# kfjahnke/envutil

Measured on AMD Instinct MI355X. Metric: Mpix/s reprojected (16K lat/lon->cubemap, b-spline-3), higher is better.
Workload: dtype f32

## Files before the change

envutil_amd/csrc/eu_render4.hip:

```cpp
#include <cstdio>
#include <cstring>
#include <vector>
#include <algorithm>
#include "eu_packed_dev.h"
#include "eu_launch.h"

#define EU4_TW 16
#define EU4_TH 8
#define EU4_WAVES 4
#ifndef EU4_WAVES0
#define EU4_WAVES0 1
#define EU4_TEXELS 384
#define EU4_OCC0 4
#endif
#define EU4_SHARDS 1024
#define EU4_WL_SHARD(s) (16 * (s))
#define EU4_WL_DONE1 (16 * EU4_SHARDS)
#define EU4_WL_DYN(x) (16 * (EU4_SHARDS + 1 + (x)))
#define EU4_WL_ENTRIES (16 * (EU4_SHARDS + 16))
#define EU4_UNIT_ROWS 4
#define EU4_COL_FLOATS 8
#define EU4_MAX_PLANS 16

__device__ __forceinline__ void eu4_box_reduce(int &mn0, int &mn1, int &mx0, int &mx1)
// ... 27 lines not shown
  unsigned keep;
  asm volatile("s_mov_b32 %0, m0\n\t"
               "s_mov_b32 m0, %1\n\t"
               "s_nop 0\n\t"
               "global_load_lds_dwordx4 %2, %3\n\t"
               "s_mov_b32 m0, %0"
               : "=&s"(keep) : "s"(dst), "v"(voff), "s"(sb) : "memory");
}

struct eu4_plan {
  const float *atab_g;
  const int *tileplan;
  const float *coltab;
  int tiles16;
  const int *l2_rows;
  int l2_off[9];
  int l2_half;
  unsigned long long l2_magic;
  const int *l1_ent;
  int l1_off[9];
  int l1_ecols;
  unsigned long long l1_magic;
  const int *xtab;
#ifdef EU5_STAMPS
  unsigned long long *stamps;
#endif
};

#ifdef EU5_STAMPS
#define EU5_STAMP(k) do { asm volatile("" ::: "memory"); st_[k] = __builtin_amdgcn_s_memtime(); asm volatile("" ::: "memory"); } while (0)
#define EU5_STAMP32(k) do { asm volatile("" ::: "memory"); st_[k] = (unsigned)__builtin_amdgcn_s_memtime(); asm volatile("" ::: "memory"); } while (0)
#else
#define EU5_STAMP(k) do { } while (0)
#define EU5_STAMP32(k) do { } while (0)
#endif

template <int NCH, int DEG, int PRJ>
__device__ __forceinline__ void eu4_tile(const eu_render_params &p, const eu4_plan &w, const float *atab,
                                         float *wtile, int tile_y, int x0, int lane)
{
  constexpr int TEX = 4;
  constexpr int order = DEG + 1;
  const eu_src_dev &s = p.src;
  const int lx = lane & 7, ly = lane >> 3;
  const int y = p.row_begin + tile_y * EU4_TH + ly;
  const bool yin = y < p.row_end;
// ... 252 lines not shown
  const int sh = gid & (EU4_SHARDS - 1);
  const int nwork = __builtin_amdgcn_readfirstlane(
    __hip_atomic_load(p.wl + EU4_WL_SHARD(sh), __ATOMIC_RELAXED, __HIP_MEMORY_SCOPE_AGENT));
  __syncthreads();
#pragma unroll 1
  for (int k = gid / EU4_SHARDS; k < nwork; k += (int)(gridDim.x * EU4_WAVES / EU4_SHARDS)) {
    const int id = __builtin_amdgcn_readfirstlane(p.wl[EU4_WL_ENTRIES + (size_t)k * EU4_SHARDS + sh]);
    const int tile_y = id / w.tiles16;
    const int x0 = (id - tile_y * w.tiles16) * EU4_TW;
    eu4_direct_tile<NCH, DEG, PRJ>(p, atab, tile_y, x0, lane);
  }
  __shared__ int last;
  __syncthreads();
  if (threadIdx.x == 0) last = atomicAdd(p.wl + EU4_WL_DONE1, 1) == (int)gridDim.x - 1;
  __syncthreads();
  if (last) {
    for (int i = threadIdx.x; i <= EU4_SHARDS + 8; i += 256)
      __hip_atomic_store(p.wl + 16 * i, 0, __ATOMIC_RELAXED, __HIP_MEMORY_SCOPE_AGENT);
  }
}

static long long eu4_followers_plan = 0, eu4_followers_last = 0;
extern "C" unsigned long long eu_hip_share_follower_tiles(void) { return (unsigned long long)eu4_followers_last; }

#ifndef EU4_DIRECT_WGS
#define EU4_DIRECT_WGS 2048
#endif

template <int NCH, int DEG, int PRJ>
static int launch4_ndp(const eu_render_params &p, const eu4_plan &w, hipStream_t st)
{
  if constexpr (PRJ == EU_SPHERICAL) {
    static const int cus = [] {
      int dev = 0, n = 0;
      if (hipGetDevice(&dev) != hipSuccess) return 0;
      if (hipDeviceGetAttribute(&n, hipDeviceAttributeMultiprocessorCount, dev) != hipSuccess) return 0;
      return n;
    }();
    const bool fast = eu_staged_fast_profile(p);
    int per_cu = 0;
    if (fast) {
      static const int occ = [] { int n = 0; return hipOccupancyMaxActiveBlocksPerMultiprocessor(&n, eu_render5_kernel<NCH, DEG, PRJ, true>, 64 * EU5_WAVES, 0) == hipSuccess ? n : 0; }();
      per_cu = occ;
    } else {
      static const int occ = [] { int n = 0; return hipOccupancyMaxActiveBlocksPerMultiprocessor(&n, eu_render5_kernel<NCH, DEG, PRJ, false>, 64 * EU5_WAVES, 0) == hipSuccess ? n : 0; }();
      per_cu = occ;
    }
    const int wgs = (cus / 8) * 8 * per_cu;
    if (wgs <= 0) return -1;
    if (fast) eu4_followers_last = eu4_followers_plan;
    if (fast) hipLaunchKernelGGL((eu_render5_kernel<NCH, DEG, PRJ, true>), dim3((unsigned)wgs), dim3(64 * EU5_WAVES), 0, st, p, w);
    else hipLaunchKernelGGL((eu_render5_kernel<NCH, DEG, PRJ, false>), dim3((unsigned)wgs), dim3(64 * EU5_WAVES), 0, st, p, w);
  } else {
    const int units = (p.tiles_y + EU4_UNIT_ROWS - 1) / EU4_UNIT_ROWS;
    dim3 grid((unsigned)(8 * ((w.tiles16 + EU4_WAVES0 - 1) / EU4_WAVES0)), (unsigned)EU4_UNIT_ROWS, (unsigned)((units + 7) / 8));
    hipLaunchKernelGGL((eu_render4s_kernel<NCH, DEG, PRJ>), grid, dim3(64 * EU4_WAVES0), 0, st, p, w);
  }
  if (hipGetLastError() != hipSuccess) return -1;
  hipLaunchKernelGGL((eu_render4d_kernel<NCH, DEG, PRJ>), dim3(EU4_DIRECT_WGS), dim3(256), 0, st, p, w);
  if (hipGetLastError() != hipSuccess) {
    (void)hipMemsetAsync(p.wl, 0, EU4_WL_ENTRIES * sizeof(int), st);
    return -1;
  }
  return 0;
}

template <int NCH, int DEG>
static int launch4_nd(const eu_render_params &p, const eu4_plan &w, hipStream_t st)
{
  switch (p.src.prj) {
    case EU_SPHERICAL: return launch4_ndp<NCH, DEG, EU_SPHERICAL>(p, w, st);
    case EU_CUBEMAP: return launch4_ndp<NCH, DEG, EU_CUBEMAP>(p, w, st);
    case EU_BIATAN6: return launch4_ndp<NCH, DEG, EU_BIATAN6>(p, w, st);
  }
// ... 1 lines not shown
}

template <int NCH>
static int launch4_n(const eu_render_params &p, const eu4_plan &w, hipStream_t st)
{
  switch (p.src.degree) {
    case 1: return launch4_nd<NCH, 1>(p, w, st);
    case 2: return launch4_nd<NCH, 2>(p, w, st);
    case 3: return launch4_nd<NCH, 3>(p, w, st);
  }
  return -2;
}

extern "C" size_t eu_render4_worklist_ints(size_t ntiles)
{
  return EU4_WL_ENTRIES + ((ntiles + EU4_SHARDS - 1) / EU4_SHARDS) * EU4_SHARDS;
}
extern "C" size_t eu_render4_worklist_header_ints(void) { return EU4_WL_ENTRIES; }

static_assert(EU_STAGED_TILE_ROWS == EU4_TH && EU_STAGED_MAX_TILES_Y == 65535 * 8 * EU4_UNIT_ROWS, "eu_select.h: eu_staged_covers");
namespace {
struct plan_cache {
  std::vector<unsigned char> key;
  eu_dev_buf<int> tileplan, l2_rows, l1_ent, xtab;
  eu_dev_buf<float> coltab;
  float *atab = nullptr;
  int planned_rows = 0;
  int l2_off[9] = {};
  int l1_off[9] = {};
  int l1_ecols = 1;
  long long follower_tiles = 0;
  hipStream_t last_stream = nullptr;
} g4s[EU_MAX_SLOTS];
#define g4 (g4s[eu_current_slot()])

bool ensure_atab()
{
  if (g4.atab) return true;
  std::vector<float> tab(768, 0.0f);
  for (int i = 0; i < EU_ATAN_TAB_ENTRIES; i++) eu_atan_tab_entry(i, tab.data() + 8 * i);
  if (hipMalloc((void **)&g4.atab, tab.size() * sizeof(float)) != hipSuccess) return false;
  return hipMemcpy(g4.atab, tab.data(), tab.size() * sizeof(float), hipMemcpyHostToDevice) == hipSuccess;
}

template <int DEG>
void launch_colplan(const eu_render_params &p, float *ct, const float *k, hipStream_t st)
{
  hipLaunchKernelGGL((eu_colplan_kernel<DEG>), dim3((unsigned)((p.width + 511) / 512)), dim3(256), 0, st, p, ct,
                     k[0], k[1], k[2], k[3]);
}

std::vector<unsigned char> eu4_plan_key(const eu_render_params &p, unsigned long long plan_gen, int share_mode)
{
  std::vector<unsigned char> key(sizeof(unsigned long long) + sizeof(eu_src_dev) + 9 * sizeof(int));
  unsigned char *q = key.data();
  memcpy(q, &plan_gen, sizeof plan_gen); q += sizeof plan_gen;
  eu_src_dev sd = p.src; sd.base = nullptr;
  memcpy(q, &sd, sizeof sd); q += sizeof sd;
  const int v[9] = { p.width, p.row_begin, p.row_end, p.band_shift, p.band_count, p.band_index, p.form, p.norm_mode, share_mode };
  memcpy(q, v, sizeof v);
  return key;
}

bool upload(eu_dev_buf<int> &buf, const std::vector<int> &v, size_t spare)
{
  if (buf.reserve(v.size() + spare) != hipSuccess) return false;
  return v.empty() || hipMemcpy(buf.p, v.data(), v.size() * sizeof(int), hipMemcpyHostToDevice) == hipSuccess;
}

int eu4_build_plans(const eu_render_params &p, int tiles16, const eu_switches &sw, const float *h_row,
                    size_t h_row_floats, hipStream_t st)
{
  std::vector<int> tp((size_t)p.tiles_y, -1);
  std::vector<float> plans;
  const bool can = p.form == EU_FORM_BA && p.norm_mode == EU_NORM_NONE && h_row;
  if (can && sw.colplan) {
    for (int ty = 0; ty < p.tiles_y; ty++) {
      float k[4] = { 0, 0, 0, 0 };
      bool same = true;
      for (int ly = 0; ly < EU4_TH && same; ly++) {
        const int y = std::min(p.row_begin + ty * EU4_TH + ly, p.row_end - 1);
        const size_t fr = (size_t)eu_frame_row(y, p.band_shift, p.band_count, p.band_index) * EU_ROW_FLOATS;
        if (fr + 6 > h_row_floats) { same = false; break; }
        const float c[4] = { h_row[fr + 0], h_row[fr + 2], h_row[fr + 3], h_row[fr + 5] };
        if (ly == 0) memcpy(k, c, sizeof k);
        else same = memcmp(k, c, sizeof k) == 0;
      }
      if (!same) continue;
      int id = -1;
      for (size_t j = 0; j < plans.size() / 4 && id < 0; j++)
// ... 2 lines not shown
        id = (int)(plans.size() / 4);
        plans.insert(plans.end(), k, k + 4);
      }
      tp[(size_t)ty] = id;
    }
  }
  const int nplans = (int)(plans.size() / 4);
  if (g4.tileplan.reserve(tp.size()) != hipSuccess) return -1;
  if (g4.coltab.reserve(std::max<size_t>(1, nplans) * (size_t)p.width * EU4_COL_FLOATS) != hipSuccess) return -1;
  if (hipStreamSynchronize(st) != hipSuccess) return -1;
  if (g4.last_stream && g4.last_stream != st && hipStreamSynchronize(g4.last_stream) != hipSuccess) return -1;
  if (hipMemcpy(g4.tileplan.p, tp.data(), tp.size() * sizeof(int), hipMemcpyHostToDevice) != hipSuccess) return -1;
  g4.planned_rows = 0;
  for (int v : tp) g4.planned_rows += v >= 0;
  auto paired = [&](int m) { return 2 * m + 1 < p.tiles_y && tp[(size_t)2 * m] >= 0 && tp[(size_t)2 * m] == tp[(size_t)2 * m + 1]; };
  {
    std::vector<int> rows[8], all;
    for (int r = 0; r < p.tiles_y; r++)
      if (!paired(r >> 1)) rows[(r / EU5_UNIT_ROWS) & 7].push_back(r);
    for (int x = 0; x < 8; x++) { g4.l2_off[x] = (int)all.size(); all.insert(all.end(), rows[x].begin(), rows[x].end()); }
    g4.l2_off[8] = (int)all.size();
    if (!upload(g4.l2_rows, all, 1)) return -1;
  }
  for (int j = 0; j < nplans; j++) {
    float *ct = g4.coltab.p + j * (size_t)p.width * EU4_COL_FLOATS;
    switch (p.src.degree) {
      case 1: launch_colplan<1>(p, ct, &plans[4 * j], st); break;
      case 2: launch_colplan<2>(p, ct, &plans[4 * j], st); break;
      default: launch_colplan<3>(p, ct, &plans[4 * j], st); break;
    }
    if (hipGetLastError() != hipSuccess) return -1;
  }
  std::vector<float> h_ct((size_t)nplans * p.width * EU4_COL_FLOATS);
  if (nplans) {
    if (hipStreamSynchronize(st) != hipSuccess) return -1;
    if (hipMemcpy(h_ct.data(), g4.coltab.p, h_ct.size() * sizeof(float), hipMemcpyDeviceToHost) != hipSuccess) return -1;
  }
  std::vector<int> cm, cp;
  for (int m = 0; 2 * m + 1 < p.tiles_y; m++)
    if (paired(m)) { cm.push_back(m); cp.push_back(tp[(size_t)2 * m]); }
  eu_share_input in;
  in.width = p.width; in.tiles16 = tiles16; in.row_begin = p.row_begin; in.row_end = p.row_end;
  in.band_mode = p.band_count > 1;
  in.ncand = (int)cm.size(); in.cand_m = cm.data(); in.cand_plan = cp.data();
  in.h_row = h_row; in.h_row_floats = h_row_floats; in.row_floats = EU_ROW_FLOATS;
  in.coltab = nplans ? h_ct.data() : nullptr; in.col_floats = EU4_COL_FLOATS; in.nplans = nplans;
// ... 2 lines not shown
  eu_share_build(in, gr);
  if (!upload(g4.l1_ent, gr.entries, 2)) return -1;
  if (g4.xtab.reserve(gr.xtab.size()) != hipSuccess) return -1;
  if (hipMemcpy(g4.xtab.p, gr.xtab.data(), gr.xtab.size() * sizeof(int), hipMemcpyHostToDevice) != hipSuccess) return -1;
  for (int x = 0; x < 9; x++) g4.l1_off[x] = gr.off[x];
  g4.l1_ecols = gr.ecols;
  g4.follower_tiles = gr.follower_tiles;
  return 0;
}

void eu4_fill_plan(eu4_plan &w)
{
  w.tileplan = g4.tileplan.p;
  w.coltab = g4.coltab.p;
  w.l2_rows = g4.l2_rows.p;
  for (int x = 0; x < 9; x++) w.l2_off[x] = g4.l2_off[x];
  w.l2_half = (w.tiles16 + 1) / 2;
  w.l2_magic = (1ull << 40) / (unsigned long long)w.l2_half + 1;
  w.l1_ent = g4.l1_ent.p;
  for (int x = 0; x < 9; x++) w.l1_off[x] = g4.l1_off[x];
  w.l1_ecols = g4.l1_ecols;
  w.l1_magic = (1ull << 40) / (unsigned long long)w.l1_ecols + 1;
  w.xtab = g4.xtab.p;
}

int launch4(const eu_render_params &p, const eu4_plan &w, hipStream_t st)
{
  switch (p.nch) {
    case 3: return launch4_n<3>(p, w, st);
    case 4: return launch4_n<4>(p, w, st);
  }
  return -2;
}

#ifdef EU5_STAMPS
int launch4_stamped(const eu_render_params &p, eu4_plan &w, hipStream_t st)
{
  static unsigned long long *d_st = nullptr; static size_t st_cap = 0; static int dumps = 0;
  const size_t ntile_st = (size_t)w.tiles16 * p.tiles_y * 8;
  const size_t nst = ntile_st + 8192 * 4;
  if (st_cap < nst) { if (d_st) (void)hipFree(d_st); if (hipMalloc((void **)&d_st, nst * 8) != hipSuccess) return -1; st_cap = nst; }
  (void)hipMemsetAsync(d_st, 0, nst * 8, st);
  w.stamps = d_st;
  const int rc_ = launch4(p, w, st);
  if (rc_ == 0 && dumps < 2 && nst >= 8 * 4096) {
    dumps++;
// ... 16 lines not shown
        const unsigned long long *q = &h[ntile_st + k * 4];
        if (!q[3]) continue;
        const double d = (double)(q[2] - q[0]);
        mn = std::min(mn, d); mx = std::max(mx, d); sum += d; l1 += (double)(q[1] - q[0]); nw++;
        first = std::min(first, (double)q[0]); last = std::max(last, (double)q[2]);
      }
      if (nw) fprintf(stderr, "eu5 waves: %zu, cycles per wave min %.0f avg %.0f max %.0f, first loop avg %.0f, first start .. last end %.0f\n",
                      nw, mn, sum / nw, mx, l1 / nw, last - first);
    }
    for (int c = 0; c < 32; c++) if (cnt[c])
      fprintf(stderr, "eu5 stamps: hoist %d npass %2d tiles %8zu | coords %7.0f box %6.0f dma-issue+weights %6.0f dma-wait %6.0f taps(all passes) %6.0f store %5.0f | tile %7.0f (100 MHz ticks? s_memtime)\n",
              c >> 4, (c & 15) - 1, cnt[c], acc[c][0] / cnt[c], acc[c][1] / cnt[c], acc[c][2] / cnt[c], acc[c][3] / cnt[c], acc[c][4] / cnt[c], acc[c][5] / cnt[c], acc[c][6] / cnt[c]);
  }
  return rc_;
}
#endif
}

extern "C" int eu_launch_render4(const eu_render_params *pp, const eu_switches *sw, const float *h_row, size_t h_row_floats,
                                 unsigned long long plan_gen, void *stream, int *launches)
{
  eu_render_params p = *pp;
  eu4_followers_last = 0;
  *launches = 2;
  if (!eu_staged_covers(p) || !p.wl) return -2;
  p.tiles_y = (p.row_end - p.row_begin + EU4_TH - 1) / EU4_TH;
  eu4_plan w;
  w.tiles16 = (p.width + EU4_TW - 1) / EU4_TW;
  if (w.tiles16 <= 0 || p.tiles_y <= 0) return 0;
  hipStream_t st = (hipStream_t)stream;
  if (!ensure_atab()) return -1;
  w.atab_g = g4.atab;
  if (p.src.prj == EU_SPHERICAL) {
    std::vector<unsigned char> key = eu4_plan_key(p, plan_gen, sw->share);
    if (key != g4.key) {
      if (eu4_build_plans(p, w.tiles16, *sw, h_row, h_row_floats, st)) return -1;
      g4.key.swap(key);
    }
    if (sw->r4 != 1 && !eu_staged_worth(p.src.degree, g4.planned_rows, p.tiles_y)) { *launches = 0; return 0; }
  }
  eu4_fill_plan(w);
  eu4_followers_plan = g4.follower_tiles;
  g4.last_stream = st;
#ifdef EU5_STAMPS
  return launch4_stamped(p, w, st);
#else
  return launch4(p, w, st);
#endif
}
```

envutil_amd/csrc/eu_render5.h:

```cpp
#define EU5_WAVES 4
#ifndef EU5_TEXELS
#define EU5_TEXELS 576
#endif
#ifndef EU5_OCC
#define EU5_OCC 4
#endif
#ifndef EU5_UNIT_ROWS
#define EU5_UNIT_ROWS 4
#endif

__device__ __forceinline__ int eu4_shard_of(int id)
{
  return (int)(((unsigned)id * 0x9E3779B1u) >> 22) & (EU4_SHARDS - 1);
}

typedef const __attribute__((address_space(3))) eu4_f4 *eu5_l4ptr;

template <int NCH, int DEG>
__device__ __forceinline__ void eu5_taps(eu_lptr lt, int a, int b, int pitch, const eu_f2 *wx, const eu_f2 *wy,
                                         eu_f2 tx, eu_f2 ty, eu_f2 &rga, eu_f2 &bxa, eu_f2 &rgb, eu_f2 &bxb)
{
  constexpr int order = DEG + 1;
  if constexpr (DEG == 1) {
    const eu_f2 wl0 = 1.0f - tx, wr0 = tx, wl1 = 1.0f - ty, wr1 = ty;
// ... 106 lines not shown
  return cc + lower;
}

__device__ __forceinline__ int eu5_out_of_range3(float a, float b, float c)
{
  const float hi = __builtin_fmaxf(__builtin_fmaxf(__builtin_fabsf(a), __builtin_fabsf(b)), __builtin_fabsf(c));
  const float lo = __builtin_fminf(__builtin_fminf(__builtin_fabsf(a), __builtin_fabsf(b)), __builtin_fabsf(c));
  return (hi <= 0x1p40f && lo >= 0x1p-40f) ? 0 : -1;
}

struct eu5_tab8 { eu_f2 c0; float A0, A1, A2, B0, B1, B2; };

template <bool FAST>
__device__ __forceinline__ void eu5_load8(const eu_render_params &p, int tile_y, int x0, int lane, eu5_tab8 &T)
{
  const int pr = lane & 3, rw = (lane >> 2) & 7, hf = lane >> 5;
  const int y = p.row_begin + tile_y * EU4_TH + rw;
  const int yc = y < p.row_end ? y : p.row_end - 1;
  const float *rt = p.row + (long long)(FAST ? yc : eu_frame_row(yc, p.band_shift, p.band_count, p.band_index)) * EU_ROW_FLOATS;
  const int xa = x0 + 8 * hf + 2 * pr, xb = xa + 1;
  const int xac = xa < p.width ? xa : p.width - 1, xbc = xb < p.width ? xb : p.width - 1;
  T.A0 = rt[0]; T.A1 = rt[1]; T.A2 = rt[2]; T.B0 = rt[3]; T.B1 = rt[4]; T.B2 = rt[5];
  T.c0 = (eu_f2){ p.col[xac], p.col[xbc] };
}

template <int NCH, int DEG, int PRJ, bool HOIST, bool FAST, bool PRE = false>
__device__ __forceinline__ void eu5_tile(const eu_render_params &p, const eu4_plan &w, const float *atab,
                                         float *wtile, const float *ct, int tile_y, int x0, int lane,
                                         const eu5_tab8 *T = nullptr, bool have_n = false, int ty_n = 0, int x0_n = 0,
                                         eu5_tab8 *Tn = nullptr)
{
  static_assert(!PRE || (!HOIST && FAST), "the prefetching form exists for plain FAST tiles");
  constexpr int TEX = 4;
  constexpr int order = DEG + 1;
  const eu_src_dev &s = p.src;
#ifdef EU5_STAMPS
  unsigned long long st_[8] = { 0, 0, 0, 0, 0, 0, 0, 0 };
#endif
  EU5_STAMP(0);
  const int pr = lane & 3, rw = (lane >> 2) & 7, hf = lane >> 5;
  const int y = p.row_begin + tile_y * EU4_TH + rw;
  const bool yin = y < p.row_end;
  const int yc = yin ? y : p.row_end - 1;
  const float *rt = p.row + (long long)(FAST ? yc : eu_frame_row(yc, p.band_shift, p.band_count, p.band_index)) * EU_ROW_FLOATS;
  const int xa = x0 + 8 * hf + 2 * pr, xb = xa + 1;
  const bool va = yin && xa < p.width, vb = yin && xb < p.width;
// ... 262 lines not shown
__device__ __forceinline__ void eu5_stage(const eu_src_dev &s, const eu5_box &bx, unsigned lds_tile, int lane)
{
  constexpr int order = DEG + 1;
  const int ibw = bx.mxx - bx.mnx + order, ibh = bx.mxy - bx.mny + order;
  const unsigned tv = eu5_divtab.v[ibw];
  const int k = (int)(tv >> 24);
  const unsigned r = ((unsigned)lane * (tv & 0x1ffffu)) >> 16, c = (unsigned)lane - r * (unsigned)ibw;
  const int bx0 = bx.mnx - DEG / 2, by0 = bx.mny - DEG / 2;
  const unsigned pitchb = (unsigned)(s.es1 * 4);
  const unsigned voff = r * pitchb + c * (NCH * 4u);
  const char *const sb0 = (const char *)(s.base + ((long long)by0 * s.es1 + (long long)bx0 * NCH));
  const unsigned long long step = (unsigned long long)k * pitchb;
  const unsigned dstep = (unsigned)(k * ibw) * 16u;
  if ((int)r < k) {
    const char *sb = sb0;
    unsigned dst = lds_tile;
#pragma unroll 1
    for (int left = ibh; left >= k; left -= k) { eu4_dma_row(dst, voff, sb); sb += step; dst += dstep; }
  }
  if ((int)r < ibh % k) {
    const int full = ibh / k;
    eu4_dma_row(lds_tile + (unsigned)full * dstep, voff, sb0 + (unsigned long long)full * step);
  }
}

struct eu5_tab16 {
  eu4_f4 a0, a1, b0, b1;
  eu_f2 c0;
  float A1A, B1A, A1B, B1B;
};

__device__ __forceinline__ void eu5_load16(const eu_render_params &p, const float *ct, int tile_y, int x0, int lane, eu5_tab16 &T)
{
  const int pr = lane & 3, rw = (lane >> 2) & 7, hf = lane >> 5;
  const int yA = p.row_begin + tile_y * EU4_TH + rw, yB = yA + EU4_TH;
  const int ycA = yA < p.row_end ? yA : p.row_end - 1, ycB = yB < p.row_end ? yB : p.row_end - 1;
  const float *rtA = p.row + (long long)ycA * EU_ROW_FLOATS, *rtB = p.row + (long long)ycB * EU_ROW_FLOATS;
  const int xa = x0 + 8 * hf + 2 * pr, xb = xa + 1;
  const int xac = xa < p.width ? xa : p.width - 1, xbc = xb < p.width ? xb : p.width - 1;
  const eu4_f4 *ea = (const eu4_f4 *)(ct + (size_t)xac * EU4_COL_FLOATS);
  const eu4_f4 *eb = (const eu4_f4 *)(ct + (size_t)xbc * EU4_COL_FLOATS);
  T.a0 = ea[0]; T.a1 = ea[1]; T.b0 = eb[0]; T.b1 = eb[1];
  T.A1A = rtA[1]; T.B1A = rtA[4]; T.A1B = rtB[1]; T.B1B = rtB[4];
  T.c0 = (eu_f2){ p.col[xac], p.col[xbc] };
}

// ... 199 lines not shown
    rx += dx; ry += dy; ul += du;
    if (rx >= tiles16) { rx -= tiles16; ry++; }
    if (ry >= UNIT) { ry -= UNIT; ul++; }
  }
  __device__ __forceinline__ bool done() const { return ul * 8 + xcd >= units; }
  __device__ __forceinline__ int row() const { return (ul * 8 + xcd) * UNIT + ry; }
  __device__ __forceinline__ int col() const
  {
    const unsigned h = ((unsigned)row() * 0x9E3779B1u) >> 16;
    int c = rx + (int)((h * (unsigned)tiles16) >> 16);
    if (c >= tiles16) c -= tiles16;
    return c;
  }
};

__device__ __forceinline__ int eu5_pair_plan(const int *tileplan, int tiles_y, int m)
{
  if (2 * m + 1 >= tiles_y) return -1;
  const eu5_cint tp = (eu5_cint)tileplan;
  const int a = tp[2 * m], b = tp[2 * m + 1];
  return a == b ? a : -1;
}

template <int NCH, int DEG, int PRJ, bool FAST>
__global__ __launch_bounds__(64 * EU5_WAVES, EU5_OCC) void eu_render5_kernel(const eu_render_params p, const eu4_plan w)
{
  __shared__ __attribute__((aligned(16))) float tile_all[EU5_WAVES * EU5_TEXELS * 4];
  __shared__ __attribute__((aligned(16))) float atab[768];
  const int lane0 = threadIdx.x & 63;
  const int wave = __builtin_amdgcn_readfirstlane(threadIdx.x >> 6);
  float *const tile = tile_all + wave * (EU5_TEXELS * 4);
  if (PRJ != EU_CUBEMAP && wave == 0) {
#pragma unroll
    for (int i = 0; i < 3; i++)
      __builtin_amdgcn_global_load_lds((eu4_gbl_void)(w.atab_g + i * 256 + lane0 * 4),
                                       (eu4_lds_void)(atab + i * 256), 16, 0, 0);
    asm volatile("s_waitcnt vmcnt(0)" ::: "memory");
  }
  __syncthreads();
#ifdef EU5_STAMPS
  const unsigned long long ws0 = __builtin_amdgcn_s_memtime();
  unsigned long long ws1 = ws0;
#endif
  const int xcd = (int)(blockIdx.x & 7);
  const int K = (int)(gridDim.x >> 3) * EU5_WAVES;
  const int t0 = (int)(blockIdx.x >> 3) * EU5_WAVES + wave;
  constexpr bool PAIRS = FAST && PRJ == EU_SPHERICAL;
// ... 21 lines not shown
#pragma unroll 1
    while (have_a) {
      const bool have_n = seek(e_n, n_n, m_n, plan_n, col_n);
      eu5_group16<NCH, DEG>(p, w, atab, tile, T, e_a, n_a, m_a, plan_a, col_a, lane0, have_n, m_n, have_n ? plan_n : 0, col_n);
      e_a = e_n; n_a = n_n; m_a = m_n; plan_a = plan_n; col_a = col_n; have_a = have_n;
    }
  }
#ifdef EU5_STAMPS
  ws1 = __builtin_amdgcn_s_memtime();
#endif
  eu5_iter<EU5_UNIT_ROWS> it;
  it.xcd = xcd; it.tiles16 = w.tiles16;
  it.units = (p.tiles_y + EU5_UNIT_ROWS - 1) / EU5_UNIT_ROWS;
  it.start(t0, K);
  if constexpr (PAIRS) {
    int *const queue = p.wl + EU4_WL_DYN(xcd);
    const int nbatch = (w.l2_off[xcd + 1] - w.l2_off[xcd]) * w.l2_half;
    const eu5_cint rows2 = (eu5_cint)w.l2_rows + w.l2_off[xcd];
    auto take = [&]() -> int {
      int v = 0;
      if (lane0 == 0) v = atomicAdd(queue, 1);
      return v;
    };
    auto decode = [&](int j, int &ty, int &tcol) -> bool {
      if (j >= nbatch) return false;
      const int r = (int)(((unsigned long long)(unsigned)j * w.l2_magic) >> 40);
      ty = rows2[r]; tcol = 2 * (j - r * w.l2_half);
      return true;
    };
    int ty_a = 0, col_a = 0, ty_n = 0, col_n = 0;
    bool have = decode(__builtin_amdgcn_readfirstlane(take()), ty_a, col_a);
    eu5_tab8 Ta, Tb;
    if (have) eu5_load8<FAST>(p, ty_a, col_a * EU4_TW, lane0, Ta);
#pragma unroll 1
    while (have) {
      const int jn_lane = take();
      const bool second = col_a + 1 < w.tiles16;
      {
        int lane = lane0;
        asm volatile("" : "+v"(lane));
        eu5_tile<NCH, DEG, PRJ, false, FAST, true>(p, w, atab, tile, nullptr, ty_a, col_a * EU4_TW, lane, &Ta, second, ty_a,
                                                   (col_a + 1) * EU4_TW, &Tb);
      }
      const bool have_n = decode(__builtin_amdgcn_readfirstlane(jn_lane), ty_n, col_n);
      if (second) {
        int lane = lane0;
        asm volatile("" : "+v"(lane));
        eu5_tile<NCH, DEG, PRJ, false, FAST, true>(p, w, atab, tile, nullptr, ty_a, (col_a + 1) * EU4_TW, lane, &Tb, have_n, ty_n,
                                                   col_n * EU4_TW, &Ta);
      } else if (have_n) eu5_load8<FAST>(p, ty_n, col_n * EU4_TW, lane0, Ta);
      ty_a = ty_n; col_a = col_n; have = have_n;
    }
  } else {
    int plan_n = (it.done() || it.row() >= p.tiles_y) ? -2 : (PRJ == EU_SPHERICAL ? ((eu5_cint)w.tileplan)[it.row()] : -1);
#pragma unroll 1
    while (!it.done()) {
      const int tile_y = it.row(), tcol = it.col(), plan = plan_n;
      it.step();
      plan_n = (it.done() || it.row() >= p.tiles_y) ? -2 : (PRJ == EU_SPHERICAL ? ((eu5_cint)w.tileplan)[it.row()] : -1);
      if (plan == -2) continue;
      int lane = lane0;
      asm volatile("" : "+v"(lane));
      if (plan >= 0)
        eu5_tile<NCH, DEG, PRJ, PRJ == EU_SPHERICAL, FAST>(p, w, atab, tile, w.coltab + (size_t)plan * p.width * EU4_COL_FLOATS,
                                                            tile_y, tcol * EU4_TW, lane);
      else
        eu5_tile<NCH, DEG, PRJ, false, FAST>(p, w, atab, tile, nullptr, tile_y, tcol * EU4_TW, lane);
    }
  }
#ifdef EU5_STAMPS
  if (lane0 == 0 && w.stamps) {
    unsigned long long *o = w.stamps + (size_t)w.tiles16 * p.tiles_y * 8 + ((size_t)blockIdx.x * EU5_WAVES + wave) * 4;
    o[0] = ws0; o[1] = ws1; o[2] = __builtin_amdgcn_s_memtime(); o[3] = 1;
  }
// ... 4 lines not shown
```

envutil_amd/csrc/eu_select.h:

```cpp
#ifndef EU_SELECT_H
#define EU_SELECT_H
#include <algorithm>
#include <climits>
#include <cstdlib>
#include <vector>
#include "eu_device.h"
#include "eu_share_groups.h"

struct eu_switches {
  int force_general;
  int hybrid;
  int r4;
  int colmajor;
  int rej;
  int colplan;
  int share;
  int direct;
  int iir_stream;
};

inline eu_switches eu_read_switches()
{
  auto first = [](const char *name) { const char *e = getenv(name); return e ? e[0] : '\0'; };
  eu_switches s;
  s.force_general = first("EU_HIP_KERNEL") == '1';
  const char hy = first("EU_HIP_HYBRID");
  s.hybrid = hy == '0' ? 0 : hy == '2' ? 2 : 1;
  const char *r4 = getenv("EU_HIP_R4");
  s.r4 = r4 ? atoi(r4) : -1;
  const char *cm = getenv("EU_HIP_COLMAJOR");
  s.colmajor = cm && cm[0] ? atoi(cm) : -1;
  const char rj = first("EU_HIP_REJ");
  s.rej = rj == '1' ? 1 : rj == '2' ? 2 : 0;
  s.colplan = first("EU_HIP_COLPLAN") != '0';
  const char sh = first("EU_HIP_SHARE");
  s.share = sh == '0' ? 0 : sh == 'm' ? EU_SHARE_MIRRORS : sh == 'f' ? EU_SHARE_FACES : EU_SHARE_FACES | EU_SHARE_MIRRORS;
  s.direct = first("EU_HIP_DIRECT") == '1';
  const char *iir = getenv("EU_HIP_IIR_STREAM");
  s.iir_stream = iir ? atoi(iir) : 7;
  return s;
}

inline bool eu_cube_source(int prj) { return prj == EU_CUBEMAP || prj == EU_BIATAN6; }

inline bool eu_packed_covers(const eu_render_params &p)
{
  if (p.stage != 0 || p.form >= EU_FORM_FISH || p.src.has_lcp || p.nch_out != p.nch) return false;
  if (p.src.prj != EU_SPHERICAL && !eu_cube_source(p.src.prj)) return false;
  if (p.src.degree < 1 || p.src.degree > 3 || p.src.es0 != p.nch) return false;
  return p.nch >= 1 && p.nch <= 4;
}

#define EU_STAGED_TILE_ROWS 8
#define EU_STAGED_MAX_TILES_Y (65535 * 8 * 4)
inline bool eu_staged_covers(const eu_render_params &p)
{
  if (!eu_packed_covers(p) || p.twine) return false;
  if (p.norm_mode != EU_NORM_NONE && p.norm_mode != EU_NORM_DIV) return false;
  if (p.nch != 3 && p.nch != 4) return false;
  if (p.src.es1 * 4 >= (1ll << 31)) return false;
  return (p.row_end - p.row_begin + EU_STAGED_TILE_ROWS - 1) / EU_STAGED_TILE_ROWS <= EU_STAGED_MAX_TILES_Y;
}
// ... 72 lines not shown
```

Before: 105,500.

## Precompute per-tile source bounding boxes in a plan-time box table

Adds a plan-time kernel that computes, for every tile of the fast lat/lon staging path, the source-pixel bounding boxes, the pass count and a work class, and stores them as packed records in a device table cached with the plan. The render kernel gets a BOXTAB variant that reads these records through scalar constant loads instead of running the per-tile coordinate/box reduction before staging. It also prefetches the next tile's record and sends dirty tiles straight to the direct worklist. This removes a serial coordinate pass and cross-lane reductions from the critical path. In exchange it costs extra memory, more register pressure from the new variant, and a plan rebuild when switches change.

```diff
diff --git a/envutil_amd/csrc/eu_render4.hip b/envutil_amd/csrc/eu_render4.hip
--- a/envutil_amd/csrc/eu_render4.hip
+++ b/envutil_amd/csrc/eu_render4.hip
@@ -73,6 +73,7 @@
   int l1_ecols;
   unsigned long long l1_magic;
   const int *xtab;
+  const int *boxtab;
 #ifdef EU5_STAMPS
   unsigned long long *stamps;
 #endif
@@ -371,6 +372,10 @@
 
 static long long eu4_followers_plan = 0, eu4_followers_last = 0;
 extern "C" unsigned long long eu_hip_share_follower_tiles(void) { return (unsigned long long)eu4_followers_last; }
+static int eu4_boxtab_last = 0;
+static long long eu4_boxtab_tiles_last = 0;
+extern "C" int eu_hip_boxtab_used(void) { return eu4_boxtab_last; }
+extern "C" unsigned long long eu_hip_boxtab_tiles(void) { return (unsigned long long)eu4_boxtab_tiles_last; }
 
 #ifndef EU4_DIRECT_WGS
 #define EU4_DIRECT_WGS 2048
@@ -387,8 +392,12 @@
       return n;
     }();
     const bool fast = eu_staged_fast_profile(p);
+    const bool bt = fast && w.boxtab != nullptr && p.out_stride < (1ll << 25);
     int per_cu = 0;
-    if (fast) {
+    if (bt) {
+      static const int occ = [] { int n = 0; return hipOccupancyMaxActiveBlocksPerMultiprocessor(&n, eu_render5_kernel<NCH, DEG, PRJ, true, true>, 64 * EU5_WAVES, 0) == hipSuccess ? n : 0; }();
+      per_cu = occ;
+    } else if (fast) {
       static const int occ = [] { int n = 0; return hipOccupancyMaxActiveBlocksPerMultiprocessor(&n, eu_render5_kernel<NCH, DEG, PRJ, true>, 64 * EU5_WAVES, 0) == hipSuccess ? n : 0; }();
       per_cu = occ;
     } else {
@@ -398,7 +407,9 @@
     const int wgs = (cus / 8) * 8 * per_cu;
     if (wgs <= 0) return -1;
     if (fast) eu4_followers_last = eu4_followers_plan;
-    if (fast) hipLaunchKernelGGL((eu_render5_kernel<NCH, DEG, PRJ, true>), dim3((unsigned)wgs), dim3(64 * EU5_WAVES), 0, st, p, w);
+    eu4_boxtab_last = bt;
+    if (bt) hipLaunchKernelGGL((eu_render5_kernel<NCH, DEG, PRJ, true, true>), dim3((unsigned)wgs), dim3(64 * EU5_WAVES), 0, st, p, w);
+    else if (fast) hipLaunchKernelGGL((eu_render5_kernel<NCH, DEG, PRJ, true>), dim3((unsigned)wgs), dim3(64 * EU5_WAVES), 0, st, p, w);
     else hipLaunchKernelGGL((eu_render5_kernel<NCH, DEG, PRJ, false>), dim3((unsigned)wgs), dim3(64 * EU5_WAVES), 0, st, p, w);
   } else {
     const int units = (p.tiles_y + EU4_UNIT_ROWS - 1) / EU4_UNIT_ROWS;
@@ -446,7 +457,9 @@
 namespace {
 struct plan_cache {
   std::vector<unsigned char> key;
-  eu_dev_buf<int> tileplan, l2_rows, l1_ent, xtab;
+  eu_dev_buf<int> tileplan, l2_rows, l1_ent, xtab, boxtab;
+  bool has_boxtab = false;
+  long long boxtab_tiles = 0;
   eu_dev_buf<float> coltab;
   float *atab = nullptr;
   int planned_rows = 0;
@@ -474,14 +487,15 @@
                      k[0], k[1], k[2], k[3]);
 }
 
-std::vector<unsigned char> eu4_plan_key(const eu_render_params &p, unsigned long long plan_gen, int share_mode)
-{
-  std::vector<unsigned char> key(sizeof(unsigned long long) + sizeof(eu_src_dev) + 9 * sizeof(int));
+std::vector<unsigned char> eu4_plan_key(const eu_render_params &p, unsigned long long plan_gen, const eu_switches &sw)
+{
+  std::vector<unsigned char> key(sizeof(unsigned long long) + sizeof(eu_src_dev) + 11 * sizeof(int));
   unsigned char *q = key.data();
   memcpy(q, &plan_gen, sizeof plan_gen); q += sizeof plan_gen;
   eu_src_dev sd = p.src; sd.base = nullptr;
   memcpy(q, &sd, sizeof sd); q += sizeof sd;
-  const int v[9] = { p.width, p.row_begin, p.row_end, p.band_shift, p.band_count, p.band_index, p.form, p.norm_mode, share_mode };
+  const int v[11] = { p.width, p.row_begin, p.row_end, p.band_shift, p.band_count, p.band_index, p.form, p.norm_mode, sw.share,
+                      sw.boxtab, sw.boxtab_max_kb };
   memcpy(q, v, sizeof v);
   return key;
 }
@@ -490,6 +504,13 @@
 {
   if (buf.reserve(v.size() + spare) != hipSuccess) return false;
   return v.empty() || hipMemcpy(buf.p, v.data(), v.size() * sizeof(int), hipMemcpyHostToDevice) == hipSuccess;
+}
+
+template <int DEG>
+void launch_boxplan(const eu_render_params &p, const float *atab_g, const int *l2_rows, int tiles16, int ntiles, int *tab, hipStream_t st)
+{
+  hipLaunchKernelGGL((eu5_boxplan_kernel<DEG>), dim3((unsigned)((ntiles + 3) / 4)), dim3(256), 0, st, p, atab_g, l2_rows, tiles16,
+                     ntiles, tab);
 }
 
 int eu4_build_plans(const eu_render_params &p, int tiles16, const eu_switches &sw, const float *h_row,
@@ -538,6 +559,23 @@
     g4.l2_off[8] = (int)all.size();
     if (!upload(g4.l2_rows, all, 1)) return -1;
   }
+  g4.has_boxtab = false; g4.boxtab_tiles = 0;
+  if (sw.boxtab && eu_staged_fast_profile(p)) {
+    const long long ntiles = (long long)g4.l2_off[8] * tiles16;
+    const long long bytes = ntiles * (EU5_BT_RECS * 16);
+    if (bytes <= (long long)sw.boxtab_max_kb * 1024) {
+      if (g4.boxtab.reserve((size_t)std::max<long long>(1, ntiles) * (EU5_BT_RECS * 4)) != hipSuccess) return -1;
+      if (ntiles > 0) {
+        switch (p.src.degree) {
+          case 1: launch_boxplan<1>(p, g4.atab, g4.l2_rows.p, tiles16, (int)ntiles, g4.boxtab.p, st); break;
+          case 2: launch_boxplan<2>(p, g4.atab, g4.l2_rows.p, tiles16, (int)ntiles, g4.boxtab.p, st); break;
+          default: launch_boxplan<3>(p, g4.atab, g4.l2_rows.p, tiles16, (int)ntiles, g4.boxtab.p, st); break;
+        }
+        if (hipGetLastError() != hipSuccess) return -1;
+      }
+      g4.has_boxtab = true; g4.boxtab_tiles = ntiles;
+    }
+  }
   for (int j = 0; j < nplans; j++) {
     float *ct = g4.coltab.p + j * (size_t)p.width * EU4_COL_FLOATS;
     switch (p.src.degree) {
@@ -586,6 +624,7 @@
   w.l1_ecols = g4.l1_ecols;
   w.l1_magic = (1ull << 40) / (unsigned long long)w.l1_ecols + 1;
   w.xtab = g4.xtab.p;
+  w.boxtab = g4.has_boxtab ? g4.boxtab.p : nullptr;
 }
 
 int launch4(const eu_render_params &p, const eu4_plan &w, hipStream_t st)
@@ -648,6 +687,7 @@
 {
   eu_render_params p = *pp;
   eu4_followers_last = 0;
+  eu4_boxtab_last = 0; eu4_boxtab_tiles_last = 0;
   *launches = 2;
   if (!eu_staged_covers(p) || !p.wl) return -2;
   p.tiles_y = (p.row_end - p.row_begin + EU4_TH - 1) / EU4_TH;
@@ -658,7 +698,7 @@
   if (!ensure_atab()) return -1;
   w.atab_g = g4.atab;
   if (p.src.prj == EU_SPHERICAL) {
-    std::vector<unsigned char> key = eu4_plan_key(p, plan_gen, sw->share);
+    std::vector<unsigned char> key = eu4_plan_key(p, plan_gen, *sw);
     if (key != g4.key) {
       if (eu4_build_plans(p, w.tiles16, *sw, h_row, h_row_floats, st)) return -1;
       g4.key.swap(key);
@@ -667,6 +707,7 @@
   }
   eu4_fill_plan(w);
   eu4_followers_plan = g4.follower_tiles;
+  eu4_boxtab_tiles_last = w.boxtab ? g4.boxtab_tiles : 0;
   g4.last_stream = st;
 #ifdef EU5_STAMPS
   return launch4_stamped(p, w, st);
diff --git a/envutil_amd/csrc/eu_render5.h b/envutil_amd/csrc/eu_render5.h
--- a/envutil_amd/csrc/eu_render5.h
+++ b/envutil_amd/csrc/eu_render5.h
@@ -152,6 +152,97 @@
   const int xac = xa < p.width ? xa : p.width - 1, xbc = xb < p.width ? xb : p.width - 1;
   T.A0 = rt[0]; T.A1 = rt[1]; T.A2 = rt[2]; T.B0 = rt[3]; T.B1 = rt[4]; T.B2 = rt[5];
   T.c0 = (eu_f2){ p.col[xac], p.col[xbc] };
+}
+
+struct eu5_co8 {
+  eu_f2 tx, ty;
+  int ixa, ixb, iya, iyb;
+  eu_i2 ok;
+};
+
+template <int DEG>
+__device__ __forceinline__ void eu5_coords8(const eu_src_dev &s, const float *atab, const eu5_tab8 &T, eu5_co8 &c)
+{
+  eu_i2 big0 = { 0, 0 }, big1 = { 0, 0 };
+  const eu_f2 c0 = T.c0;
+  const eu_f2 rx = T.B0 * c0 + T.A0, ry = T.B1 * c0 + T.A1, rz = T.B2 * c0 + T.A2;
+  const eu_i2 ok = { ~eu5_out_of_range3(rx.x, ry.x, rz.x), ~eu5_out_of_range3(rx.y, ry.y, rz.y) };
+  const eu_f2 q2 = rx * rx + rz * rz;
+  const eu_f2 qs = eu_sqrt2_safe(q2);
+  const eu_f2 lat = eu_atan2f_2_lean(ry, qs, atab, 1, big0);
+  const eu_f2 lon = eu_atan2f_2_lean(rx, rz, atab, 0, big1);
+  c.ok = ok & ~(big0 | big1);
+  eu_f2 i0 = { (float)((double)lon.x - s.tex_x0), (float)((double)lon.y - s.tex_x0) };
+  if (s.cdiv_ok) i0 = eu_div2_const(i0, s.ext_w, s.rcp_ext_w);
+  else i0 = eu_div2_rr(i0, s.ext_w, eu_rcp_refined(s.ext_w));
+  i0 = i0 * s.total_w; i0 = i0 - .5f;
+  const eu_f2 sx = i0 - s.win_x_off;
+  const eu_f2 gx = eu5_gate2(sx, s.gate0, s.lower0, s.upper0);
+  eu_f2 fx;
+  if constexpr (DEG & 1) fx = (eu_f2){ floorf(gx.x), floorf(gx.y) };
+  else fx = (eu_f2){ roundf(gx.x), roundf(gx.y) };
+  c.tx = gx - fx;
+  c.ixa = (int)fx.x; c.ixb = (int)fx.y;
+  eu_f2 i1 = { (float)((double)lat.x - s.tex_y0), (float)((double)lat.y - s.tex_y0) };
+  if (s.cdiv_ok) i1 = eu_div2_const(i1, s.ext_h, s.rcp_ext_h);
+  else i1 = eu_div2_rr(i1, s.ext_h, eu_rcp_refined(s.ext_h));
+  i1 = i1 * s.total_h; i1 = i1 - .5f;
+  const eu_f2 sy = i1 - s.win_y_off;
+  c.ty = eu5_gate2(sy, s.gate1, s.lower1, s.upper1);
+}
+
+template <int DEG>
+__device__ __forceinline__ void eu5_split_y(eu5_co8 &c)
+{
+  const eu_f2 gy = c.ty;
+  eu_f2 fy;
+  if constexpr (DEG & 1) fy = (eu_f2){ floorf(gy.x), floorf(gy.y) };
+  else fy = (eu_f2){ roundf(gy.x), roundf(gy.y) };
+  c.ty = gy - fy;
+  c.iya = (int)fy.x; c.iyb = (int)fy.y;
+}
+
+struct eu5_boxes {
+  int q0, q1, q2, q3, h0, h1, h2, h3;
+  eu5_box full;
+  int npass;
+  bool clean;
+};
+
+template <int DEG, bool GATES>
+__device__ __forceinline__ void eu5_box_stage(int gate0, int gate1, float upper0, float upper1, eu_i2 hit, eu_i2 ok,
+                                              int ixa, int ixb, int iya, int iyb, eu5_boxes &b)
+{
+  constexpr int order = DEG + 1;
+  int q0 = INT_MAX, q1 = INT_MAX, q2 = INT_MIN, q3 = INT_MIN, h0, h1, h2, h3;
+  if (hit.x) { q0 = ixa; q2 = ixa; q1 = iya; q3 = iya; }
+  if (hit.y) { q0 = min(q0, ixb); q2 = max(q2, ixb); q1 = min(q1, iyb); q3 = max(q3, iyb); }
+  eu5_box_reduce(q0, q1, q2, q3, h0, h1, h2, h3);
+  const eu5_box full = eu5_box_join(eu5_box_at(h0, h1, h2, h3, 31), eu5_box_at(h0, h1, h2, h3, 63));
+  bool clean = __ballot((hit.x && !ok.x) || (hit.y && !ok.y)) == 0ull;
+  if constexpr (GATES) {
+    const int cw = (int)(upper0 + 0.5f), ch = (int)(upper1 + 0.5f);
+    if (full.mnx != INT_MAX) {
+      if (gate0 == 2 && full.mnx < 0) clean = false;
+      if (gate0 != 0 && full.mxx >= cw - 1) clean = false;
+      if (gate1 == 2 && full.mny < 0) clean = false;
+      if (gate1 != 0 && full.mxy >= ch - 1) clean = false;
+    }
+  }
+  int npass = 1;
+  const int f = eu5_box_fits<order>(full);
+  if (f < 0) npass = 0;
+  else if (f == 0) {
+    npass = 2;
+    if (eu5_box_fits<order>(eu5_box_at(h0, h1, h2, h3, 31)) == 0 || eu5_box_fits<order>(eu5_box_at(h0, h1, h2, h3, 63)) == 0) {
+      npass = 4;
+      if (eu5_box_fits<order>(eu5_box_at(q0, q1, q2, q3, 15)) == 0 || eu5_box_fits<order>(eu5_box_at(q0, q1, q2, q3, 31)) == 0 ||
+          eu5_box_fits<order>(eu5_box_at(q0, q1, q2, q3, 47)) == 0 || eu5_box_fits<order>(eu5_box_at(q0, q1, q2, q3, 63)) == 0)
+        npass = -1;
+    }
+  }
+  b.q0 = q0; b.q1 = q1; b.q2 = q2; b.q3 = q3; b.h0 = h0; b.h1 = h1; b.h2 = h2; b.h3 = h3;
+  b.full = full; b.npass = npass; b.clean = clean;
 }
 
 template <int NCH, int DEG, int PRJ, bool HOIST, bool FAST, bool PRE = false>
@@ -460,6 +551,173 @@
     const int full = ibh / k;
     eu4_dma_row(lds_tile + (unsigned)full * dstep, voff, sb0 + (unsigned long long)full * step);
   }
+}
+
+#define EU5_BT_RECS 4
+#define EU5_BT_WORK 8
+#define EU5_WAIT_VM0 0x0F70
+typedef unsigned eu5_u3 __attribute__((ext_vector_type(3)));
+typedef unsigned eu5_u4 __attribute__((ext_vector_type(4)));
+typedef int eu5_i4 __attribute__((ext_vector_type(4)));
+typedef const __attribute__((address_space(4))) eu5_i4 *eu5_crec;
+
+__device__ __forceinline__ int eu5_bt_pack(const eu5_box &b, int w3, int c)
+{
+  if (c == 2) return b.mnx == INT_MAX ? -1 : (int)(((unsigned)b.mxx - (unsigned)b.mnx) | (((unsigned)b.mxy - (unsigned)b.mny) << 16));
+  return c == 0 ? b.mnx : c == 1 ? b.mny : w3;
+}
+
+template <int DEG>
+__global__ __launch_bounds__(256) void eu5_boxplan_kernel(const eu_render_params p, const float *atab_g, const int *l2_rows,
+                                                          int tiles16, int ntiles, int *tab)
+{
+  __shared__ __attribute__((aligned(16))) float atab[768];
+  const int lane = threadIdx.x & 63;
+  const int wave = __builtin_amdgcn_readfirstlane(threadIdx.x >> 6);
+  if (wave == 0) {
+#pragma unroll
+    for (int i = 0; i < 3; i++)
+      __builtin_amdgcn_global_load_lds((eu4_gbl_void)(atab_g + i * 256 + lane * 4), (eu4_lds_void)(atab + i * 256), 16, 0, 0);
+    asm volatile("s_waitcnt vmcnt(0)" ::: "memory");
+  }
+  __syncthreads();
+  const int g = (int)blockIdx.x * 4 + wave;
+  if (g >= ntiles) return;
+  const int slot = g / tiles16, tcol = g - slot * tiles16;
+  const int tile_y = __builtin_amdgcn_readfirstlane(l2_rows[slot]);
+  const int x0 = tcol * EU4_TW;
+  const eu_src_dev &s = p.src;
+  const int pr = lane & 3, rw = (lane >> 2) & 7, hf = lane >> 5;
+  const int y = p.row_begin + tile_y * EU4_TH + rw;
+  const bool yin = y < p.row_end;
+  const int xa = x0 + 8 * hf + 2 * pr, xb = xa + 1;
+  const bool va = yin && xa < p.width, vb = yin && xb < p.width;
+  eu5_tab8 T;
+  eu5_load8<true>(p, tile_y, x0, lane, T);
+  eu5_co8 c;
+  eu5_coords8<DEG>(s, atab, T, c);
+  eu5_split_y<DEG>(c);
+  const eu_i2 hit = { va ? -1 : 0, vb ? -1 : 0 };
+  eu5_boxes B;
+  eu5_box_stage<DEG, true>(s.gate0, s.gate1, s.upper0, s.upper1, hit, c.ok, c.ixa, c.ixb, c.iya, c.iyb, B);
+  const int cls = (B.npass < 0 || (B.npass > 0 && !B.clean)) ? EU5_BT_WORK : B.npass;
+  eu5_box r[EU5_BT_RECS] = { B.full, B.full, B.full, B.full };
+  if (B.npass == 2) { r[0] = eu5_box_at(B.h0, B.h1, B.h2, B.h3, 31); r[1] = eu5_box_at(B.h0, B.h1, B.h2, B.h3, 63); }
+  if (B.npass == 4) {
+#pragma unroll
+    for (int k = 0; k < 4; k++) r[k] = eu5_box_at(B.q0, B.q1, B.q2, B.q3, 15 + 16 * k);
+  }
+  int v = 0;
+#pragma unroll
+  for (int k = 0; k < EU5_BT_RECS; k++) {
+#pragma unroll
+    for (int i = 0; i < 4; i++)
+      if (lane == 4 * k + i) v = eu5_bt_pack(r[k], k == 0 ? cls : 0, i);
+  }
+  if (lane < 4 * EU5_BT_RECS) tab[(size_t)g * (4 * EU5_BT_RECS) + lane] = v;
+}
+
+template <int NCH, int DEG>
+__device__ __forceinline__ void eu5_tile_bt(const eu_render_params &p, const eu4_plan &w, const float *atab, float *wtile,
+                                            int tile_y, int x0, int lane, const eu5_tab8 &T, eu5_i4 R, eu5_crec rec,
+                                            bool have_n, int ty_n, int x0_n, eu5_tab8 &Tn)
+{
+  constexpr int order = DEG + 1;
+  const eu_src_dev &s = p.src;
+#ifdef EU5_STAMPS
+  unsigned long long st_[8] = { 0, 0, 0, 0, 0, 0, 0, 0 };
+#endif
+  EU5_STAMP(0);
+  const int cls = R.w;
+  if (cls & EU5_BT_WORK) {
+    if (lane == 0) {
+      const int id = tile_y * w.tiles16 + x0 / EU4_TW;
+      const int sh = eu4_shard_of(id);
+      const int slot = atomicAdd(p.wl + EU4_WL_SHARD(sh), 1);
+      p.wl[EU4_WL_ENTRIES + (size_t)slot * EU4_SHARDS + sh] = id;
+    }
+    if (have_n) eu5_load8<true>(p, ty_n, x0_n, lane, Tn);
+    __builtin_amdgcn_s_waitcnt(EU5_WAIT_VM0);
+    return;
+  }
+  const int npass = cls & 7;
+  const unsigned lds_tile = (unsigned)(unsigned long long)(eu4_lds_void)wtile;
+  eu5_tab8 Tl = T;
+  asm volatile("" : "+v"(Tl.c0), "+v"(Tl.A0), "+v"(Tl.A1), "+v"(Tl.A2), "+v"(Tl.B0), "+v"(Tl.B1), "+v"(Tl.B2));
+  eu5_box bx = { R.x, R.y, R.x + (R.z & 0xffff), R.y + (R.z >> 16) };
+  bool some = npass > 0 && R.z >= 0;
+  if (some) eu5_stage<NCH, DEG>(s, bx, lds_tile, lane);
+  const int pr = lane & 3, rw = (lane >> 2) & 7, hf = lane >> 5;
+  const int y = p.row_begin + tile_y * EU4_TH + rw;
+  const bool yin = y < p.row_end;
+  const int xa = x0 + 8 * hf + 2 * pr, xb = xa + 1;
+  const bool va = yin && xa < p.width, vb = yin && xb < p.width;
+  eu_f2 rga = { 0.0f, 0.0f }, bxa = { 0.0f, 0.0f }, rgb = { 0.0f, 0.0f }, bxb = { 0.0f, 0.0f };
+  if (npass > 0) {
+    eu5_co8 c;
+    eu5_coords8<DEG>(s, atab, Tl, c);
+    eu5_split_y<DEG>(c);
+#ifdef EU5_STAMPS
+    asm volatile("" : : "v"(c.iya), "v"(c.iyb), "v"(c.ixa), "v"(c.ixb));
+#endif
+    EU5_STAMP(2);
+#ifdef EU5_STAMPS
+    st_[3] = st_[2];
+#endif
+    eu_f2 wx[order], wy[order];
+    if constexpr (DEG >= 2) {
+      eu_weights2<DEG>(s.wm, c.ty, wy);
+      eu_weights2<DEG>(s.wm, c.tx, wx);
+    }
+    const int grp = npass == 1 ? 0 : npass == 2 ? hf : (lane >> 4);
+#pragma unroll 1
+    for (int pi = 0; pi < npass; pi++) {
+      eu5_i4 Rn = { 0, 0, -1, 0 };
+      if (pi + 1 < npass) Rn = rec[pi + 1];
+      if (some) {
+        if (pi > 0) eu5_stage<NCH, DEG>(s, bx, lds_tile, lane);
+        const int ibw = bx.mxx - bx.mnx + order;
+        const bool mine = grp == pi;
+        const int oa = (mine && va) ? ((c.iya - bx.mny) * ibw + (c.ixa - bx.mnx)) * 4 : 0;
+        const int ob = (mine && vb) ? ((c.iyb - bx.mny) * ibw + (c.ixb - bx.mnx)) * 4 : 0;
+        if (pi == 0) EU5_STAMP(4);
+        asm volatile("s_waitcnt vmcnt(0)" ::: "memory");
+        if (pi == 0) EU5_STAMP(5);
+        if (mine) eu5_taps<NCH, DEG>((eu_lptr)wtile, oa, ob, ibw * 4, wx, wy, c.tx, c.ty, rga, bxa, rgb, bxb);
+      }
+      bx = (eu5_box){ Rn.x, Rn.y, Rn.x + (Rn.z & 0xffff), Rn.y + (Rn.z >> 16) };
+      some = Rn.z >= 0;
+    }
+  }
+#ifdef EU5_STAMPS
+  asm volatile("" : : "v"(rga), "v"(bxa), "v"(rgb), "v"(bxb));
+#endif
+  EU5_STAMP(6);
+  float qa[4] = { rga.x, rga.y, bxa.x, bxa.y }, qb[4] = { rgb.x, rgb.y, bxb.x, bxb.y };
+  if (have_n) eu5_load8<true>(p, ty_n, x0_n, lane, Tn);
+  __builtin_amdgcn_sched_barrier(0);
+  {
+    float *const base = p.out + (long long)(tile_y * EU4_TH) * p.out_stride + (long long)x0 * NCH;
+    const __amdgpu_buffer_rsrc_t rs = __builtin_amdgcn_make_buffer_rsrc(base, 0, 0x80000000u, 0x00027000);
+    const unsigned off = ((unsigned)rw * (unsigned)p.out_stride + (unsigned)((8 * hf + 2 * pr) * NCH)) * 4u;
+    const unsigned oa = va ? off : 0xfffff000u, ob = vb ? oa + NCH * 4u : 0xfffff000u;
+    if constexpr (NCH == 3) {
+      __builtin_amdgcn_raw_buffer_store_b96((eu5_u3){ __float_as_uint(qa[0]), __float_as_uint(qa[1]), __float_as_uint(qa[2]) }, rs, (int)oa, 0, 0);
+      __builtin_amdgcn_raw_buffer_store_b96((eu5_u3){ __float_as_uint(qb[0]), __float_as_uint(qb[1]), __float_as_uint(qb[2]) }, rs, (int)ob, 0, 0);
+    } else {
+      __builtin_amdgcn_raw_buffer_store_b128((eu5_u4){ __float_as_uint(qa[0]), __float_as_uint(qa[1]), __float_as_uint(qa[2]), __float_as_uint(qa[3]) }, rs, (int)oa, 0, 0);
+      __builtin_amdgcn_raw_buffer_store_b128((eu5_u4){ __float_as_uint(qb[0]), __float_as_uint(qb[1]), __float_as_uint(qb[2]), __float_as_uint(qb[3]) }, rs, (int)ob, 0, 0);
+    }
+  }
+  EU5_STAMP(7);
+#ifdef EU5_STAMPS
+  if (lane == 0 && w.stamps) {
+    unsigned long long *o = w.stamps + ((size_t)tile_y * w.tiles16 + x0 / EU4_TW) * 8;
+    st_[1] = (unsigned long long)(npass + 1);
+#pragma unroll
+    for (int k = 0; k < 8; k++) o[k] = st_[k];
+  }
+#endif
 }
 
 struct eu5_tab16 {
@@ -705,7 +963,7 @@
   return a == b ? a : -1;
 }
 
-template <int NCH, int DEG, int PRJ, bool FAST>
+template <int NCH, int DEG, int PRJ, bool FAST, bool BOXTAB = false>
 __global__ __launch_bounds__(64 * EU5_WAVES, EU5_OCC) void eu_render5_kernel(const eu_render_params p, const eu4_plan w)
 {
   __shared__ __attribute__((aligned(16))) float tile_all[EU5_WAVES * EU5_TEXELS * 4];
@@ -773,34 +1031,76 @@
       if (lane0 == 0) v = atomicAdd(queue, 1);
       return v;
     };
-    auto decode = [&](int j, int &ty, int &tcol) -> bool {
-      if (j >= nbatch) return false;
-      const int r = (int)(((unsigned long long)(unsigned)j * w.l2_magic) >> 40);
-      ty = rows2[r]; tcol = 2 * (j - r * w.l2_half);
-      return true;
-    };
-    int ty_a = 0, col_a = 0, ty_n = 0, col_n = 0;
-    bool have = decode(__builtin_amdgcn_readfirstlane(take()), ty_a, col_a);
-    eu5_tab8 Ta, Tb;
-    if (have) eu5_load8<FAST>(p, ty_a, col_a * EU4_TW, lane0, Ta);
+    if constexpr (BOXTAB) {
+      static_assert(FAST && PRJ == EU_SPHERICAL, "the box table is that of the FAST lat/lon second loop");
+      const eu5_crec bt = (eu5_crec)w.boxtab;
+      auto decode = [&](int j, int &ty, int &tcol, int &ti) -> bool {
+        if (j >= nbatch) return false;
+        const int r = (int)(((unsigned long long)(unsigned)j * w.l2_magic) >> 40);
+        ty = rows2[r]; tcol = 2 * (j - r * w.l2_half);
+        ti = ((w.l2_off[xcd] + r) * w.tiles16 + tcol) * EU5_BT_RECS;
+        return true;
+      };
+      int ty_a = 0, col_a = 0, ti_a = 0, ty_n = 0, col_n = 0, ti_n = 0;
+      bool have = decode(__builtin_amdgcn_readfirstlane(take()), ty_a, col_a, ti_a);
+      eu5_tab8 Ta, Tb;
+      eu5_i4 Ra = { 0, 0, -1, 0 }, Rb = { 0, 0, -1, 0 };
+      if (have) { Ra = bt[ti_a]; eu5_load8<FAST>(p, ty_a, col_a * EU4_TW, lane0, Ta); }
+      __builtin_amdgcn_s_waitcnt(EU5_WAIT_VM0);
 #pragma unroll 1
-    while (have) {
-      const int jn_lane = take();
-      const bool second = col_a + 1 < w.tiles16;
-      {
-        int lane = lane0;
-        asm volatile("" : "+v"(lane));
-        eu5_tile<NCH, DEG, PRJ, false, FAST, true>(p, w, atab, tile, nullptr, ty_a, col_a * EU4_TW, lane, &Ta, second, ty_a,
-                                                   (col_a + 1) * EU4_TW, &Tb);
-      }
-      const bool have_n = decode(__builtin_amdgcn_readfirstlane(jn_lane), ty_n, col_n);
-      if (second) {
-        int lane = lane0;
-        asm volatile("" : "+v"(lane));
-        eu5_tile<NCH, DEG, PRJ, false, FAST, true>(p, w, atab, tile, nullptr, ty_a, (col_a + 1) * EU4_TW, lane, &Tb, have_n, ty_n,
-                                                   col_n * EU4_TW, &Ta);
-      } else if (have_n) eu5_load8<FAST>(p, ty_n, col_n * EU4_TW, lane0, Ta);
-      ty_a = ty_n; col_a = col_n; have = have_n;
+      while (have) {
+        const int jn_lane = take();
+        const bool second = col_a + 1 < w.tiles16;
+        if (second) Rb = bt[ti_a + EU5_BT_RECS];
+        {
+          int lane = lane0;
+          asm volatile("" : "+v"(lane));
+          eu5_tile_bt<NCH, DEG>(p, w, atab, tile, ty_a, col_a * EU4_TW, lane, Ta, Ra, bt + ti_a, second, ty_a,
+                                (col_a + 1) * EU4_TW, Tb);
+        }
+        const bool have_n = decode(__builtin_amdgcn_readfirstlane(jn_lane), ty_n, col_n, ti_n);
+        if (have_n) Ra = bt[ti_n];
+        if (second) {
+          int lane = lane0;
+          asm volatile("" : "+v"(lane));
+          eu5_tile_bt<NCH, DEG>(p, w, atab, tile, ty_a, (col_a + 1) * EU4_TW, lane, Tb, Rb, bt + ti_a + EU5_BT_RECS, have_n,
+                                ty_n, col_n * EU4_TW, Ta);
+        } else if (have_n) {
+          eu5_load8<FAST>(p, ty_n, col_n * EU4_TW, lane0, Ta);
+          __builtin_amdgcn_s_waitcnt(EU5_WAIT_VM0);
+        }
+        ty_a = ty_n; col_a = col_n; ti_a = ti_n; have = have_n;
+      }
+    } else {
+      auto decode = [&](int j, int &ty, int &tcol) -> bool {
+        if (j >= nbatch) return false;
+        const int r = (int)(((unsigned long long)(unsigned)j * w.l2_magic) >> 40);
+        ty = rows2[r]; tcol = 2 * (j - r * w.l2_half);
+        return true;
+      };
+      int ty_a = 0, col_a = 0, ty_n = 0, col_n = 0;
+      bool have = decode(__builtin_amdgcn_readfirstlane(take()), ty_a, col_a);
+      eu5_tab8 Ta, Tb;
+      if (have) eu5_load8<FAST>(p, ty_a, col_a * EU4_TW, lane0, Ta);
+  #pragma unroll 1
+      while (have) {
+        const int jn_lane = take();
+        const bool second = col_a + 1 < w.tiles16;
+        {
+          int lane = lane0;
+          asm volatile("" : "+v"(lane));
+          eu5_tile<NCH, DEG, PRJ, false, FAST, true>(p, w, atab, tile, nullptr, ty_a, col_a * EU4_TW, lane, &Ta, second, ty_a,
+                                                     (col_a + 1) * EU4_TW, &Tb);
+        }
+        const bool have_n = decode(__builtin_amdgcn_readfirstlane(jn_lane), ty_n, col_n);
+        if (second) {
+          int lane = lane0;
+          asm volatile("" : "+v"(lane));
+          eu5_tile<NCH, DEG, PRJ, false, FAST, true>(p, w, atab, tile, nullptr, ty_a, (col_a + 1) * EU4_TW, lane, &Tb, have_n, ty_n,
+                                                     col_n * EU4_TW, &Ta);
+        } else if (have_n) eu5_load8<FAST>(p, ty_n, col_n * EU4_TW, lane0, Ta);
+        ty_a = ty_n; col_a = col_n; have = have_n;
+      }
     }
   } else {
     int plan_n = (it.done() || it.row() >= p.tiles_y) ? -2 : (PRJ == EU_SPHERICAL ? ((eu5_cint)w.tileplan)[it.row()] : -1);
diff --git a/envutil_amd/csrc/eu_select.h b/envutil_amd/csrc/eu_select.h
--- a/envutil_amd/csrc/eu_select.h
+++ b/envutil_amd/csrc/eu_select.h
@@ -17,7 +17,11 @@
   int share;
   int direct;
   int iir_stream;
+  int boxtab;
+  int boxtab_max_kb;
 };
+
+#define EU_BOXTAB_MAX_KB 65536
 
 inline eu_switches eu_read_switches()
 {
@@ -38,6 +42,9 @@
   s.direct = first("EU_HIP_DIRECT") == '1';
   const char *iir = getenv("EU_HIP_IIR_STREAM");
   s.iir_stream = iir ? atoi(iir) : 7;
+  s.boxtab = first("EU_HIP_BOXTAB") != '0';
+  const char *bm = getenv("EU_HIP_BOXTAB_MAX_KB");
+  s.boxtab_max_kb = bm && bm[0] ? std::max(0, std::min(atoi(bm), 16 * 1024 * 1024)) : EU_BOXTAB_MAX_KB;
   return s;
 }
 
```

Result: faster. 109,900, median of 6 (+4.2%).
